# monkey0head/RePlay_cql

Measured on AMD Instinct MI355X. Metric: CQL train-steps/sec, higher is better.
Workload: dtype bf16; 1 GPU; BASELINE.json configs[2]: synthetic 1000000 users x 100000 items, CQL d=128, L=50, B=4096/GPU, bf16 MFMA + fp32 accumulate; users=1000000, items=100000, d=128, window=50, batch_per_gpu=4096, global_batch=4096, parallelism=dp1 (users sharded by rank, RCCL gradient all-reduce), k=10, dp_variant=single

## Files before the change

### replay_cql_amd/csrc/common.h

```cpp
#pragma once
#include <hip/hip_runtime.h>
#include <stdint.h>
#include <stdio.h>
#include <stdarg.h>

#include "../../include/cqlrec.h"

typedef __attribute__((ext_vector_type(8))) __bf16 bf16x8;
typedef __attribute__((ext_vector_type(4))) __bf16 bf16x4;
typedef __attribute__((ext_vector_type(16))) float f32x16;
typedef __attribute__((ext_vector_type(4))) float f32x4;
typedef __attribute__((address_space(3))) bf16x4 lds_bf16x4;

#define CQL_WAVE 64
#define CQL_LOG2E 1.4426950408889634f
#define CQL_LN2 0.6931471805599453f
#define NEG_INF_F (-__builtin_inff())

void cql_set_error(const char* fmt, ...);
#define CQL_REQUIRE(cond, ...)            \
  do {                                    \
    if (!(cond)) {                        \
      cql_set_error(__VA_ARGS__);         \
      return CQLREC_ERR_INVALID;          \
// ... 56 lines not shown
}
__device__ __forceinline__ uint32_t pack_bf16x2(float lo, float hi) {
  return (uint32_t)f32_to_bf16_bits(lo) | ((uint32_t)f32_to_bf16_bits(hi) << 16);
}

__device__ __forceinline__ int mfma_row(int reg, int half) { return (reg & 3) + 8 * (reg >> 2) + 4 * half; }

template <int D>
__device__ __forceinline__ int swz_chunk(int row, int ch) {
  if constexpr (D == 64) return ch ^ ((row >> 1) & 7);
  else return ch ^ (row & 15);
}

__device__ __forceinline__ float fast_exp2(float x) { return __builtin_amdgcn_exp2f(x); }

__device__ __forceinline__ uint32_t f32_order_key(float f) {
  uint32_t u = __float_as_uint(f);
  return (u & 0x80000000u) ? ~u : (u | 0x80000000u);
}
__device__ __forceinline__ float f32_from_order_key(uint32_t k) {
  uint32_t u = (k & 0x80000000u) ? (k & 0x7FFFFFFFu) : ~k;
  return __uint_as_float(u);
}

struct CqlAdamFix {
  int valid;
  const float* slab;
  const float* slab_cs;
  int32_t G, T, nblk, items, D;
  float scale;
  int64_t n_items;
  int64_t rows_off, cs_off;
};
int cql_adam_ema_fix(float* theta, float* grads, float* m, float* v, float* target, uint16_t* theta_b, uint16_t* target_b,
                     int64_t n, float step_size, float sqrt_bc2, float beta1, float beta2, float eps, float tau,
                     int32_t zero_grads, const CqlAdamFix* fix, hipStream_t stream);
#define CQL_ADAM_DEFER_CAP 64
struct CqlAdamSteps {
  float step_size[CQL_ADAM_DEFER_CAP], sqrt_bc2[CQL_ADAM_DEFER_CAP];
};
int cql_adam_ema_rows_deferred(float* theta, float* grads, float* m, float* v, float* target, uint16_t* theta_b,
                               uint16_t* target_b, int64_t n, const CqlAdamSteps& tab, uint64_t step, float beta1, float beta2,
                               float eps, float tau, int32_t zero_grads, const uint8_t* row_map, const uint8_t* read_next,
                               uint8_t* age, int32_t d, int64_t n_rows, hipStream_t stream);
int cql_mark_read_rows(const int64_t* offsets, const int32_t* items, const int32_t* users, const int32_t* tpos,
                       int64_t n_states, int32_t L, int64_t n_items, uint8_t* read_map, hipStream_t s);
int cql_gather_pool_bwd_mark_rows(const void* ws, int64_t n_states, int32_t L, int32_t d, int64_t n_items, uint8_t* row_map,
                                  hipStream_t s);
```

### replay_cql_amd/csrc/gbwd.hip

```cpp
#include <cstring>
#include <rocprim/device/device_radix_sort.hpp>

#include "common.h"

__global__ __launch_bounds__(256) void gbwd_pairs_kernel(const int64_t* __restrict__ offsets,
                                                         const int32_t* __restrict__ items,
                                                         const int32_t* __restrict__ users,
                                                         const int32_t* __restrict__ ends, int end_delta,
                                                         int64_t n_states, int L, uint32_t pad_key,
                                                         uint32_t* __restrict__ keys, uint32_t* __restrict__ vals,
                                                         int32_t* __restrict__ lens) {
  const int lane = threadIdx.x & 63;
  const int64_t state = (int64_t)blockIdx.x * 4 + (threadIdx.x >> 6);
  if (state >= n_states) return;
  const int u = users[state];
  const int64_t o0 = offsets[u];
  const int end = ends ? (ends[state] + end_delta) : (int)(offsets[u + 1] - o0);
  const int len = end < L ? end : L;
  if (lane == 0) lens[state] = len;
  const int32_t* win = items + o0 + end - len;
  for (int j = lane; j < L; j += 64) {
    keys[state * L + j] = (j < len) ? (uint32_t)win[j] : pad_key;
    vals[state * L + j] = (uint32_t)state;
  }
}

__global__ __launch_bounds__(256) void gbwd_scale_kernel(const float4* __restrict__ dh0, const int32_t* __restrict__ lens,
                                                         int64_t n4, int d4, float4* __restrict__ g) {
  const int64_t i = (int64_t)blockIdx.x * blockDim.x + threadIdx.x;
  if (i >= n4) return;
  const int len = lens[i / d4];
  const float fl = (float)len;
  const float4 v = dh0[i];
  g[i] = len > 0 ? make_float4(v.x / fl, v.y / fl, v.z / fl, v.w / fl) : make_float4(0.f, 0.f, 0.f, 0.f);
}

template <int D, bool SRC_BF16>
__device__ __forceinline__ void segsum_add_row(float (&acc)[D / 64], float& accw, const void* __restrict__ src,
                                               const float* __restrict__ w, uint32_t row, int lane) {
  constexpr int PER = D / 64;
  if constexpr (SRC_BF16) {
    const float wt = w[row];
    const uint16_t* h = (const uint16_t*)src + (int64_t)row * D;
#pragma unroll
    for (int k = 0; k < PER; ++k) acc[k] += wt * bf16_bits_to_f32(h[k * 64 + lane]);
    accw += wt;
  } else {
    const float* g = (const float*)src + (int64_t)row * D;
#pragma unroll
    for (int k = 0; k < PER; ++k) acc[k] += g[k * 64 + lane];
  }
}

template <int D, bool SRC_BF16, int CH>
__global__ __launch_bounds__(256) void segsum_pass1_kernel(const void* __restrict__ src, const float* __restrict__ w,
                                                           const uint32_t* __restrict__ keys,
                                                           const uint32_t* __restrict__ vals, int64_t n_pairs,
                                                           uint32_t pad_key, float* __restrict__ dst,
                                                           float* __restrict__ dst_w, float* __restrict__ edge,
                                                           float* __restrict__ edge_w, int accumulate) {
  constexpr int PER = D / 64;
  const int lane = threadIdx.x & 63;
  const int64_t chunk = (int64_t)blockIdx.x * 4 + (threadIdx.x >> 6);
  const int64_t chunk0 = chunk * CH;
  if (chunk0 >= n_pairs) return;
  const int64_t idx = chunk0 + lane;
  const bool mine = lane < CH && idx < n_pairs;
  const uint32_t my_key = mine ? keys[idx] : pad_key;
  const uint32_t my_val = mine ? vals[idx] : 0u;
  if (__builtin_amdgcn_readfirstlane(my_key) == pad_key) return;
  const uint32_t prev_key = (chunk0 > 0) ? keys[chunk0 - 1] : pad_key;
  const uint32_t next_key = (chunk0 + CH < n_pairs) ? keys[chunk0 + CH] : pad_key;
  float acc[PER], accw = 0.f;
#pragma unroll
  for (int k = 0; k < PER; ++k) acc[k] = 0.f;
  uint32_t run_key = __builtin_amdgcn_readfirstlane(my_key);
  bool open_left = (run_key == prev_key);
  auto flush = [&](bool open_right) {
    float* row;
    float* roww = nullptr;
    if (open_left) { row = edge + (chunk * 2 + 0) * D; if (SRC_BF16) roww = edge_w + chunk * 2 + 0; }
    else if (open_right) { row = edge + (chunk * 2 + 1) * D; if (SRC_BF16) roww = edge_w + chunk * 2 + 1; }
    else { row = dst + (int64_t)run_key * D; if (SRC_BF16) roww = dst_w + run_key; }
    const bool add = accumulate && row != edge + (chunk * 2 + 0) * D && row != edge + (chunk * 2 + 1) * D;
#pragma unroll
    for (int k = 0; k < PER; ++k) row[k * 64 + lane] = add ? row[k * 64 + lane] + acc[k] : acc[k];
    if (SRC_BF16 && lane == 0) *roww = add ? *roww + accw : accw;
  };
#pragma unroll 8
  for (int j = 0; j < CH; ++j) {
    const uint32_t kj = __shfl(my_key, j);
    if (kj != run_key) {
      flush(false);
#pragma unroll
      for (int k = 0; k < PER; ++k) acc[k] = 0.f;
      accw = 0.f;
      run_key = kj;
      open_left = false;
      if (kj == pad_key) return;
    }
    segsum_add_row<D, SRC_BF16>(acc, accw, src, w, __shfl(my_val, j), lane);
  }
  flush(run_key == next_key);
}

template <int D, bool SRC_BF16, int CH>
__global__ __launch_bounds__(256) void segsum_pass2_kernel(const uint32_t* __restrict__ keys, int64_t n_pairs,
                                                           uint32_t pad_key, const float* __restrict__ edge,
                                                           const float* __restrict__ edge_w, float* __restrict__ dst,
                                                           float* __restrict__ dst_w, int accumulate) {
  constexpr int PER = D / 64;
  const int lane = threadIdx.x & 63;
  const int64_t c = (int64_t)blockIdx.x * 4 + (threadIdx.x >> 6);
  const int64_t n_chunks = (n_pairs + CH - 1) / CH;
  if (c + 1 >= n_chunks) return;
  auto key_at = [&](int64_t i) { return i < n_pairs ? keys[i] : pad_key; };
  const uint32_t k = key_at(c * CH + CH - 1);
  if (k == pad_key || key_at((c + 1) * CH) != k) return;
  if (key_at(c * CH) == k && c > 0 && key_at(c * CH - 1) == k) return;
  int64_t lo = (c + 1) * CH, hi = n_pairs;
  while (lo < hi) {
    const int64_t mid = (lo + hi) >> 1;
    if (keys[mid] == k) lo = mid + 1; else hi = mid;
  }
  const int64_t j_end = (lo - 1) / CH;
  float acc[PER], accw = 0.f;
#pragma unroll
  for (int q = 0; q < PER; ++q) acc[q] = edge[(c * 2 + 1) * D + q * 64 + lane];
  if (SRC_BF16) accw = edge_w[c * 2 + 1];
#pragma unroll 4
  for (int64_t j = c + 1; j <= j_end; ++j) {
#pragma unroll
    for (int q = 0; q < PER; ++q) acc[q] += edge[(j * 2 + 0) * D + q * 64 + lane];
    if (SRC_BF16) accw += edge_w[j * 2 + 0];
  }
#pragma unroll
  for (int q = 0; q < PER; ++q) {
    float* o = dst + (int64_t)k * D + q * 64 + lane;
    *o = accumulate ? *o + acc[q] : acc[q];
  }
  if (SRC_BF16 && lane == 0) dst_w[k] = accumulate ? dst_w[k] + accw : accw;
}

template <bool SRC_BF16, int CH>
static void segsum_launch(const void* src, const float* w, const uint32_t* keys, const uint32_t* vals, int64_t n_pairs,
                          uint32_t pad_key, int d, float* dst, float* dst_w, float* edge, float* edge_w, hipStream_t s,
                          int accumulate = 0) {
  dim3 grid(cql_ceil_div((n_pairs + CH - 1) / CH, 4)), block(256);
#define SS1(DD) hipLaunchKernelGGL((segsum_pass1_kernel<DD, SRC_BF16, CH>), grid, block, 0, s, src, w, keys, vals, n_pairs, pad_key, dst, dst_w, edge, edge_w, accumulate)
#define SS2(DD) hipLaunchKernelGGL((segsum_pass2_kernel<DD, SRC_BF16, CH>), grid, block, 0, s, keys, n_pairs, pad_key, edge, edge_w, dst, dst_w, accumulate)
  if (d == 64) { SS1(64); SS2(64); } else if (d == 128) { SS1(128); SS2(128); } else { SS1(256); SS2(256); }
#undef SS1
#undef SS2
}

#define GB_CH 64
#define OH_CH 8

static inline int64_t a256(int64_t x) { return (x + 255) / 256 * 256; }
static inline unsigned key_bits(int64_t n_items) {
  unsigned b = 1;
  while ((1ll << b) <= n_items) ++b;
  return b;
}
static int64_t sort_temp_bound(int64_t n) { return a256(2 * n * 4 * 2) + (8ll << 20); }

namespace {
struct GbWs {
  float* g;
  float* edge;
  int32_t* lens;
  uint32_t *keys_in, *vals_in, *keys_out, *vals_out;
  void* temp;
  size_t temp_cap;
  int64_t total;
};
GbWs gb_carve(void* ws, int64_t n_states, int32_t L, int32_t d) {
  const int64_t n = n_states * L;
  char* p = (char*)ws;
  GbWs w;
  w.g = (float*)p;              p += a256(n_states * d * 4);
  w.edge = (float*)p;           p += a256(((n + GB_CH - 1) / GB_CH) * 2 * d * 4);
  w.lens = (int32_t*)p;         p += a256(n_states * 4);
// ... 168 lines not shown
int cql_onehot_prepare(const int32_t* act, int64_t batch, int64_t n_items, int32_t d, void* ws, int64_t ws_bytes,
                       hipStream_t s) {
  CQL_REQUIRE(act && ws, "onehot_prepare: NULL pointer");
  CQL_REQUIRE(batch > 0 && ws_bytes >= cql_onehot_ws_bytes(batch, d), "onehot_prepare: workspace too small");
  const OhWs w = oh_carve(ws, batch, d);
  CqlProfScope prof(CQLREC_PH_GATHER_BWD, s);
  hipLaunchKernelGGL(onehot_pairs_kernel, dim3(cql_ceil_div(batch, 256)), dim3(256), 0, s, act, batch, w.keys_in, w.vals_in);
  size_t need = 0;
  hipError_t e = rocprim::radix_sort_pairs(nullptr, need, w.keys_in, w.keys_out, w.vals_in, w.vals_out, (size_t)batch, 0u,
                                           key_bits(n_items), s);
  if (e != hipSuccess || need > w.temp_cap) {
    cql_set_error("onehot_prepare: radix sort needs %zu bytes of scratch (have %zu), err=%d", need, w.temp_cap, (int)e);
    return CQLREC_ERR_HIP;
  }
  e = rocprim::radix_sort_pairs(w.temp, need, w.keys_in, w.keys_out, w.vals_in, w.vals_out, (size_t)batch, 0u,
                                key_bits(n_items), s);
  if (e != hipSuccess) {
    cql_set_error("onehot_prepare: radix sort failed: %s", hipGetErrorString(e));
    return CQLREC_ERR_HIP;
  }
  CQL_LAUNCH_CHECK("onehot_prepare");
  return CQLREC_OK;
}

int cql_onehot_apply(const float* coef, const uint16_t* H_b, int64_t batch, int64_t n_items, int32_t d, void* ws,
                     float* g_E_out, float* g_b_out, hipStream_t s, int accumulate) {
  CQL_REQUIRE(coef && H_b && ws && g_E_out && g_b_out, "onehot_apply: NULL pointer");
  const OhWs w = oh_carve(ws, batch, d);
  CqlProfScope prof(CQLREC_PH_QHEAD_SMALL, s);
  segsum_launch<true, OH_CH>(H_b, coef, w.keys_out, w.vals_out, batch, (uint32_t)n_items, d, g_E_out, g_b_out, w.edge, w.edge_w, s, accumulate);
  CQL_LAUNCH_CHECK("onehot_apply");
  return CQLREC_OK;
}
```

### replay_cql_amd/csrc/misc.hip

```cpp
#include <stdlib.h>
#include "common.h"
#include "adam_math.h"

static thread_local char g_err[512] = "";
void cql_set_error(const char* fmt, ...) {
  va_list ap;
  va_start(ap, fmt);
  vsnprintf(g_err, sizeof(g_err), fmt, ap);
  va_end(ap);
}
extern "C" const char* cqlrec_last_error(void) { return g_err; }
extern "C" int cqlrec_abi_version(void) { return CQLREC_ABI_VERSION; }

#define CQL_PROF_POOL 8192
static struct {
  bool on = false;
  bool created = false;
  hipEvent_t ev[CQL_PROF_POOL][2];
  int phase[CQL_PROF_POOL];
  int n = 0;
  int open = -1;
  uint32_t mask = 0xFFFFFFFFu;
} g_prof;

// ... 732 lines not shown
      st4<NT>(theta + i, p[0], p[1], p[2], p[3]);
      st4<NT>(m + i, mm[0], mm[1], mm[2], mm[3]);
      st4<NT>(v + i, vv[0], vv[1], vv[2], vv[3]);
      st4<NT>(target + i, tt[0], tt[1], tt[2], tt[3]);
      theta_b[i] = make_uint2(pack_bf16x2(p[0], p[1]), pack_bf16x2(p[2], p[3]));
      target_b[i] = make_uint2(pack_bf16x2(tt[0], tt[1]), pack_bf16x2(tt[2], tt[3]));
    }
    if (zero_grads) st4<NT>(grads + i, 0.f, 0.f, 0.f, 0.f);
  }
}

int cql_adam_ema_rows_deferred(float* theta, float* grads, float* m, float* v, float* target, uint16_t* theta_b,
                               uint16_t* target_b, int64_t n, const CqlAdamSteps& tab, uint64_t step, float beta1, float beta2,
                               float eps, float tau, int32_t zero_grads, const uint8_t* row_map, const uint8_t* read_next,
                               uint8_t* age, int32_t d, int64_t n_rows, hipStream_t stream) {
  CQL_REQUIRE(theta && grads && m && v && target && theta_b && target_b && row_map && age,
              "adam_ema_rows_deferred: NULL pointer");
  CQL_REQUIRE(n > 0 && n % 4 == 0, "adam_ema_rows_deferred: n=%lld must be a positive multiple of 4", (long long)n);
  CQL_REQUIRE(d == 64 || d == 128 || d == 256, "adam_ema_rows_deferred: d=%d unsupported", d);
  CQL_REQUIRE(n_rows >= 0 && n_rows * d <= n, "adam_ema_rows_deferred: %lld rows of %d do not fit n=%lld", (long long)n_rows,
              d, (long long)n);
  const int64_t n4 = n / 4;
  int blocks = (int)((n4 + 255) / 256);
  if (blocks > 8192) blocks = 8192;
  CqlProfScope prof(CQLREC_PH_ADAM, stream);
  hipLaunchKernelGGL(adam_ema_rows_deferred_kernel<true>, dim3(blocks), dim3(256), 0, stream, (float4*)theta, (float4*)grads,
                     (float4*)m, (float4*)v, (float4*)target, (uint2*)theta_b, (uint2*)target_b, n4, tab, (uint32_t)step,
                     beta1, beta2, eps, tau, zero_grads, row_map, read_next, age, __builtin_ctz((unsigned)d) - 2, n_rows);
  CQL_LAUNCH_CHECK("adam_ema (deferred rows)");
  return CQLREC_OK;
}

__device__ __forceinline__ void adam_fix4(const CqlAdamFix& f, float (&g)[4], int64_t i4, int ld, int li) {
  const int64_t e = 4 * i4;
  uint32_t item;
  int col = -1;
  if (e >= f.rows_off && e < f.rows_off + f.n_items * f.D) {
    const uint64_t r = (uint64_t)(e - f.rows_off);
    item = (uint32_t)(r >> ld);
    col = (int)(r & (uint64_t)(f.D - 1));
  } else if (e >= f.cs_off && e < f.cs_off + f.n_items) {
    item = (uint32_t)(e - f.cs_off);
  } else {
    return;
  }
#ifdef ADAMFIX_ABL_NOLOOP
  return;
#endif
  const uint32_t grp = item >> li, row = item & (uint32_t)(f.items - 1);
  const uint32_t W = (uint32_t)f.G * (uint32_t)f.T, nblk = (uint32_t)f.nblk, lo = grp * (uint32_t)f.T, hi = lo + (uint32_t)f.T;
  for (uint32_t p = ((lo + 1) * nblk + W - 1) / W; p < nblk; ++p) {
    const uint32_t u0 = (uint32_t)((uint64_t)p * W / nblk);
    if (u0 >= hi) break;
    if (u0 <= lo) continue;
    if ((uint32_t)(((uint64_t)p + 1) * W / nblk) == u0) continue;
    if (col >= 0) {
      const float4 s4 = *reinterpret_cast<const float4*>(f.slab + ((int64_t)p * f.items + row) * f.D + col);
      g[0] += f.scale * s4.x; g[1] += f.scale * s4.y; g[2] += f.scale * s4.z; g[3] += f.scale * s4.w;
    } else {
      const float* sc = f.slab_cs + (int64_t)p * f.items + row;
#pragma unroll
      for (int k = 0; k < 4; ++k)
        if ((int64_t)item + k < f.n_items) g[k] += f.scale * sc[k];
    }
  }
}

template <bool NT>
__global__ __launch_bounds__(256) void adam_ema_fix_kernel(float4* __restrict__ theta, float4* __restrict__ grads,
                                                           float4* __restrict__ m, float4* __restrict__ v,
                                                           float4* __restrict__ target, uint2* __restrict__ theta_b,
                                                           uint2* __restrict__ target_b, int64_t n4, float step_size,
                                                           float sqrt_bc2, float beta1, float beta2, float eps, float tau,
                                                           int zero_grads, CqlAdamFix fix) {
  const float omb1 = 1.0f - beta1, omb2 = 1.0f - beta2, omt = 1.0f - tau;
  const int ld = __builtin_ctz((unsigned)fix.D), li = __builtin_ctz((unsigned)fix.items);
  for (int64_t i = (int64_t)blockIdx.x * blockDim.x + threadIdx.x; i < n4; i += (int64_t)gridDim.x * blockDim.x) {
    const float4 g4 = ld4<NT>(grads + i);
    float4 p4 = ld4<NT>(theta + i), m4 = ld4<NT>(m + i), v4 = ld4<NT>(v + i), t4 = ld4<NT>(target + i);
    float g[4] = {g4.x, g4.y, g4.z, g4.w};
    adam_fix4(fix, g, i, ld, li);
    float p[4] = {p4.x, p4.y, p4.z, p4.w}, mm[4] = {m4.x, m4.y, m4.z, m4.w}, vv[4] = {v4.x, v4.y, v4.z, v4.w},
          tt[4] = {t4.x, t4.y, t4.z, t4.w};
#pragma unroll
    for (int k = 0; k < 4; ++k) {
      adam_ema_elem(g[k], p[k], mm[k], vv[k], tt[k], step_size, sqrt_bc2, beta1, beta2, eps, tau, omb1, omb2, omt);
    }
    st4<NT>(theta + i, p[0], p[1], p[2], p[3]);
    st4<NT>(m + i, mm[0], mm[1], mm[2], mm[3]);
    st4<NT>(v + i, vv[0], vv[1], vv[2], vv[3]);
    st4<NT>(target + i, tt[0], tt[1], tt[2], tt[3]);
    theta_b[i] = make_uint2(pack_bf16x2(p[0], p[1]), pack_bf16x2(p[2], p[3]));
    target_b[i] = make_uint2(pack_bf16x2(tt[0], tt[1]), pack_bf16x2(tt[2], tt[3]));
    if (zero_grads) st4<NT>(grads + i, 0.f, 0.f, 0.f, 0.f);
  }
}

int cql_adam_ema_fix(float* theta, float* grads, float* m, float* v, float* target, uint16_t* theta_b, uint16_t* target_b,
                     int64_t n, float step_size, float sqrt_bc2, float beta1, float beta2, float eps, float tau,
                     int32_t zero_grads, const CqlAdamFix* fix, hipStream_t stream) {
  const bool pow2 = fix && fix->valid && (fix->D & (fix->D - 1)) == 0 && (fix->items & (fix->items - 1)) == 0 &&
                    fix->rows_off % 4 == 0 && fix->cs_off % 4 == 0 &&
                    (int64_t)fix->G * fix->T * ((int64_t)fix->nblk + 1) < (1ll << 31) && fix->n_items < (1ll << 31);
  CQL_REQUIRE(!fix || !fix->valid || pow2, "adam_ema: deferred fix-up outside the supported range");
  if (!fix || !fix->valid)
    return cqlrec_adam_ema(theta, grads, m, v, target, theta_b, target_b, n, step_size, sqrt_bc2, beta1, beta2, eps, tau,
                           zero_grads, (cqlrec_stream)stream);
  CQL_REQUIRE(theta && grads && m && v && target && theta_b && target_b, "adam_ema: NULL pointer");
  CQL_REQUIRE(n > 0 && n % 4 == 0, "adam_ema: n=%lld must be a positive multiple of 4", (long long)n);
  const int64_t n4 = n / 4;
  int blocks = (int)((n4 + 255) / 256);
  if (blocks > 8192) blocks = 8192;
  CqlProfScope prof(CQLREC_PH_ADAM, stream);
  hipLaunchKernelGGL(adam_ema_fix_kernel<true>, dim3(blocks), dim3(256), 0, stream, (float4*)theta, (float4*)grads,
                     (float4*)m, (float4*)v, (float4*)target, (uint2*)theta_b, (uint2*)target_b, n4, step_size, sqrt_bc2,
                     beta1, beta2, eps, tau, zero_grads, *fix);
  CQL_LAUNCH_CHECK("adam_ema (deferred fix-up)");
  return CQLREC_OK;
}

extern "C" int cqlrec_adam_ema(float* theta, float* grads, float* m, float* v, float* target, uint16_t* theta_b,
                               uint16_t* target_b, int64_t n, float step_size, float sqrt_bc2, float beta1, float beta2,
                               float eps, float tau, int32_t zero_grads, cqlrec_stream stream) {
  CQL_REQUIRE(theta && grads && m && v && target && theta_b && target_b, "adam_ema: NULL pointer");
  CQL_REQUIRE(n > 0 && n % 4 == 0, "adam_ema: n=%lld must be a positive multiple of 4", (long long)n);
  const int64_t n4 = n / 4;
  int blocks = (int)((n4 + 255) / 256);
  if (blocks > 8192) blocks = 8192;
  CqlProfScope prof(CQLREC_PH_ADAM, (hipStream_t)stream);
  hipLaunchKernelGGL(adam_ema_kernel<true>, dim3(blocks), dim3(256), 0, (hipStream_t)stream, (float4*)theta,
                     (float4*)grads, (float4*)m, (float4*)v, (float4*)target, (uint2*)theta_b, (uint2*)target_b, n4,
                     step_size, sqrt_bc2, beta1, beta2, eps, tau, zero_grads);
  CQL_LAUNCH_CHECK("adam_ema");
  return CQLREC_OK;
}

__global__ __launch_bounds__(256) void cast_bf16_kernel(const float4* __restrict__ src, uint2* __restrict__ dst,
                                                        int64_t n4) {
  for (int64_t i = (int64_t)blockIdx.x * blockDim.x + threadIdx.x; i < n4; i += (int64_t)gridDim.x * blockDim.x) {
    const float4 p = src[i];
    dst[i] = make_uint2(pack_bf16x2(p.x, p.y), pack_bf16x2(p.z, p.w));
  }
}
extern "C" int cqlrec_cast_bf16(const float* src, uint16_t* dst_b, int64_t n, cqlrec_stream stream) {
  CQL_REQUIRE(src && dst_b, "cast_bf16: NULL pointer");
  CQL_REQUIRE(n > 0 && n % 4 == 0, "cast_bf16: n=%lld must be a positive multiple of 4", (long long)n);
  const int64_t n4 = n / 4;
  int blocks = (int)((n4 + 255) / 256);
  if (blocks > 8192) blocks = 8192;
// ... 6 lines not shown
```

### replay_cql_amd/csrc/train.hip

```cpp
#include <math.h>
#include <stdlib.h>
#include "common.h"
#include "qhead_internal.h"

static int g_concurrency = -1;

enum { MK_LOSS = 0, MK_DH, MK_DE, MK_CHAIN, MK_ADAM_IN, MK_ADAM_OUT, MK_PROLOGUE, MK_LSE, MK_NEXT_LOSS, MK_ENC_DX, MK_GATHER_BWD, MK_SORT_NEXT, MK_COUNT };
static hipEvent_t g_marks[MK_COUNT];
static int g_marks_on = 0;
static int g_mark_phase = 0;
static void mark(int k, hipStream_t s) {
  if (g_marks_on && g_mark_phase) (void)hipEventRecord(g_marks[k], s);
}
extern "C" int cqlrec_debug_marks_enable(int32_t on) {
  if (on && !g_marks[0])
    for (int i = 0; i < MK_COUNT; ++i)
      if (hipEventCreate(&g_marks[i]) != hipSuccess) return CQLREC_ERR_HIP;
  g_marks_on = on ? 1 : 0;
  return CQLREC_OK;
}
extern "C" int cqlrec_debug_marks_read(float* ms_out) {
  if (!g_marks[0] || !ms_out) return CQLREC_ERR_INVALID;
  for (int i = 0; i < MK_COUNT; ++i) {
    ms_out[i] = -1.f;
    if (hipEventSynchronize(g_marks[i]) != hipSuccess) continue;
    float ms = 0.f;
    if (hipEventElapsedTime(&ms, g_marks[MK_LOSS], g_marks[i]) == hipSuccess) ms_out[i] = ms;
  }
  return CQLREC_OK;
}

namespace {
struct Carve {
  char* base;
  int64_t off;
  explicit Carve(void* p) : base((char*)p), off(0) {}
  template <typename T>
  T* take(int64_t n) {
    T* p = base ? (T*)(base + off) : nullptr;
    off += (n * (int64_t)sizeof(T) + 255) / 256 * 256;
    return p;
  }
};

struct StepWs {
  int32_t *users, *tpos, *act, *a_star;
  float *rew, *done, *q_a, *lse, *nlse2, *nlse_nat, *q_targ, *y, *coef, *maxv, *loss, *term;
  float *h0_s, *dH, *dh0;
  uint16_t *h0b, *zb, *hb, *h0b_t, *zb_t, *hb_t;
  void *ws_q, *ws_q2, *ws_qb, *ws_qb2, *ws_enc, *ws_gb, *ws_oh;
  uint8_t* row_map;
  uint8_t* read_map;
  uint8_t* age;
  int64_t ws_q_bytes, ws_qb_bytes, ws_qf_bytes, ws_enc_bytes, ws_gb_bytes, ws_oh_bytes;
  int64_t total;
};

void carve_small(Carve& c, StepWs& w, int32_t B, int32_t d) {
  w.users = c.take<int32_t>(B);
  w.tpos = c.take<int32_t>(B);
  w.act = c.take<int32_t>(B);
  w.a_star = c.take<int32_t>(B);
  w.rew = c.take<float>(B);
  w.done = c.take<float>(B);
  w.q_a = c.take<float>(B);
  w.lse = c.take<float>(B);
  w.nlse2 = c.take<float>(B);
  w.nlse_nat = c.take<float>(B);
  w.q_targ = c.take<float>(B);
  w.y = c.take<float>(B);
  w.coef = c.take<float>(B);
  w.maxv = c.take<float>(B);
  w.loss = c.take<float>(64);
  w.term = c.take<float>(B);
  w.h0_s = c.take<float>((int64_t)B * d);
  w.dH = c.take<float>((int64_t)B * d);
  w.dh0 = c.take<float>((int64_t)B * d);
  w.h0b = c.take<uint16_t>((int64_t)2 * B * d);
  w.zb = c.take<uint16_t>((int64_t)2 * B * d);
  w.hb = c.take<uint16_t>((int64_t)2 * B * d);
  w.h0b_t = c.take<uint16_t>((int64_t)B * d);
  w.zb_t = c.take<uint16_t>((int64_t)B * d);
  w.hb_t = c.take<uint16_t>((int64_t)B * d);
}

StepWs carve_step(void* ws, int32_t B, int64_t N, int32_t d, int32_t L, uint64_t step = 0) {
  StepWs w, other;
  Carve c(ws);
  if (step & 1) {
    carve_small(c, other, B, d);
    carve_small(c, w, B, d);
  } else {
    carve_small(c, w, B, d);
    carve_small(c, other, B, d);
  }
  w.ws_q_bytes = cqlrec_qhead_ws_bytes(B, N, d);
  w.ws_q = c.take<char>(w.ws_q_bytes);
  w.ws_q2 = c.take<char>(w.ws_q_bytes);
  w.ws_qb_bytes = cqlrec_qhead_bwd_ws_bytes(B, N, d);
  w.ws_qf_bytes = w.ws_qb_bytes + w.ws_q_bytes;
  w.ws_qb = c.take<char>(w.ws_qf_bytes);
  w.ws_qb2 = c.take<char>(w.ws_qb_bytes);
  w.ws_enc_bytes = cqlrec_encoder_bwd_ws_bytes(B, d);
  w.ws_enc = c.take<char>(w.ws_enc_bytes);
  w.ws_gb_bytes = cqlrec_gather_pool_bwd_ws_bytes(B, L, d);
  void* gb0 = c.take<char>(w.ws_gb_bytes);
  void* gb1 = c.take<char>(w.ws_gb_bytes);
  w.ws_gb = (step & 1) ? gb1 : gb0;
  w.ws_oh_bytes = cql_onehot_ws_bytes(B, d);
  void* oh0 = c.take<char>(w.ws_oh_bytes);
  void* oh1 = c.take<char>(w.ws_oh_bytes);
  w.ws_oh = (step & 1) ? oh1 : oh0;
  uint8_t* rm0 = c.take<uint8_t>(N);
  uint8_t* rm1 = c.take<uint8_t>(N);
  w.row_map = (step & 1) ? rm1 : rm0;
  uint8_t* rd0 = c.take<uint8_t>(N);
  uint8_t* rd1 = c.take<uint8_t>(N);
  w.read_map = (step & 1) ? rd1 : rd0;
  w.age = c.take<uint8_t>(N);
  w.total = c.off;
  return w;
}

int check_ctx(const cqlrec_train_ctx* c) {
  CQL_REQUIRE(c != nullptr, "train_step: ctx is NULL");
  CQL_REQUIRE(c->offsets && c->items && c->rewards, "train_step: CSR pointers are NULL");
  CQL_REQUIRE(c->theta && c->grads && c->adam_m && c->adam_v && c->target && c->theta_b && c->target_b,
              "train_step: model state pointers are NULL");
  CQL_REQUIRE(c->ws != nullptr, "train_step: workspace is NULL");
  CQL_REQUIRE(c->batch > 0 && c->window > 0 && c->world > 0 && c->rank >= 0 && c->rank < c->world,
              "train_step: batch=%d window=%d world=%d rank=%d", c->batch, c->window, c->world, c->rank);
  const int32_t d = c->layout.d;
  CQL_REQUIRE(d == 64 || d == 128 || d == 256, "train_step: d=%d unsupported", d);
  CQL_REQUIRE(c->ws_bytes >= cqlrec_train_ws_bytes(c->batch, c->layout.n_items, d, c->window),
              "train_step: workspace too small");
  return CQLREC_OK;
}
}

extern "C" int cqlrec_set_concurrency(int32_t on) {
  g_concurrency = on ? 1 : 0;
  return CQLREC_OK;
}

extern "C" int64_t cqlrec_train_ws_bytes(int32_t batch, int64_t n_items, int32_t d, int32_t window) {
  return carve_step(nullptr, batch, n_items, d, window).total + 256;
}

#define CQL_TRY(expr)            \
  do {                           \
    int rc__ = (expr);           \
    if (rc__ != CQLREC_OK) return rc__; \
// ... 278 lines not shown
  CQL_TRY(cql_qhead_argmax_step(w.hb + Bd, B, p.Eout_b, p.b_out, N, d, w.ws_q2, w.ws_q_bytes, w.maxv, w.a_star, (hipStream_t)sb));
  CQL_TRY(cqlrec_gather_dot(w.hb_t, p.tEout_b, p.tb_out, w.a_star, B, d, w.q_targ, sb));
  if (par && (hipEventRecord(ss.join2, ss.s2) != hipSuccess || hipStreamWaitEvent(s, ss.join2, 0) != hipSuccess)) {
    cql_set_error("train_step_forward: joining the forward branches failed");
    return CQLREC_ERR_HIP;
  }
  const float inv_batch = 1.0f / ((float)B * (float)c->world);
  CQL_TRY(cql_td_coef(w.q_a, w.lse, w.q_targ, w.rew, w.done, B, (float)c->gamma, (float)c->alpha, inv_batch, w.coef, w.y,
                      w.term, s));
  if (loss_sum_deferred) *loss_sum_deferred = true;
  else CQL_TRY(cql_td_loss_sum(w.term, B, inv_batch, loss_out ? loss_out : w.loss, s));
  if (g_mark_phase == 2) mark(MK_NEXT_LOSS, s);
  return CQLREC_OK;
}

int backward_items_long_impl(const cqlrec_train_ctx* c, uint64_t step, cqlrec_stream stream, CqlAdamFix* fix) {
  const cqlrec_layout& L = c->layout;
  const int32_t B = c->batch, d = L.d;
  StepWs w = carve_step(c->ws, B, L.n_items, d, c->window, step);
  const StepPtrs p = step_ptrs(c);
  return cql_qhead_bwd_items_long(w.hb, w.nlse2, w.coef, w.act, B, p.Eout_b, p.b_out, L.n_items, d, alpha_scale(c), w.ws_qb2,
                                  w.ws_qb_bytes, c->grads + L.off_E_out, c->grads + L.off_b_out, (hipStream_t)stream, fix,
                                  w.nlse_nat);
}
int backward_items_onehot_impl(const cqlrec_train_ctx* c, uint64_t step, cqlrec_stream stream) {
  const cqlrec_layout& L = c->layout;
  const int32_t B = c->batch, d = L.d;
  StepWs w = carve_step(c->ws, B, L.n_items, d, c->window, step);
  SideStream& ss = side_stream();
  if (ss.ok) CQL_HIP_TRY(hipStreamWaitEvent((hipStream_t)stream, ss.sorted[step & 1], 0), "train_step_backward_items");
  return cql_onehot_apply(w.coef, w.hb, B, L.n_items, d, w.ws_oh, c->grads + L.off_E_out, c->grads + L.off_b_out,
                          (hipStream_t)stream, 1);
}
int backward_items_impl(const cqlrec_train_ctx* c, uint64_t step, cqlrec_stream stream, CqlAdamFix* defer = nullptr) {
  const cqlrec_layout& L = c->layout;
  CqlAdamFix fix = {};
  CQL_TRY(backward_items_long_impl(c, step, stream, &fix));
  CQL_TRY(backward_items_onehot_impl(c, step, stream));
  if (defer) *defer = fix;
  else CQL_TRY(cql_qde_fixup_deferred(fix, c->grads + L.off_E_out, c->grads + L.off_b_out, (hipStream_t)stream));
  return CQLREC_OK;
}

int backward_states_impl(const cqlrec_train_ctx* c, uint64_t step, cqlrec_stream stream) {
  const cqlrec_layout& L = c->layout;
  const int32_t B = c->batch, d = L.d;
  const int64_t N = L.n_items;
  StepWs w = carve_step(c->ws, B, N, d, c->window, step);
  const StepPtrs p = step_ptrs(c);
  CQL_TRY(cql_qhead_dh_finish(w.ws_qb, B, N, d, w.lse, w.coef, w.act, p.Eout_b, alpha_scale(c), w.dH,
                              (hipStream_t)stream, 2));
  SideStream& ss = side_stream();
  if (ss.ok) CQL_HIP_TRY(hipEventRecord(ss.dh, (hipStream_t)stream), "train_step_backward_rest");
  return CQLREC_OK;
}

int backward_chain_impl(const cqlrec_train_ctx* c, uint64_t step, cqlrec_stream stream) {
  const cqlrec_layout& L = c->layout;
  const int32_t B = c->batch, d = L.d, W = c->window;
  const int64_t N = L.n_items;
  StepWs w = carve_step(c->ws, B, N, d, W, step);
  const StepPtrs p = step_ptrs(c);
  SideStream& ss = side_stream();
  hipStream_t s = (hipStream_t)stream;
  const bool split = ss.ok && ss.s2 && ss.s2 != s;
  CQL_TRY(cql_encoder_bwd_parts(w.dH, w.zb, w.h0b, p.W1_b, p.W2_b, B, d, w.ws_enc, w.ws_enc_bytes, c->grads + L.off_W1,
// ... 50 lines not shown
extern "C" int cqlrec_train_step_backward_items(const cqlrec_train_ctx* c, uint64_t step, cqlrec_stream stream) {
  CQL_TRY(check_ctx(c));
  if (g_early_long[step & 1]) {
    g_early_long[step & 1] = false;
    const cqlrec_layout& L = c->layout;
    CQL_TRY(backward_items_onehot_impl(c, step, stream));
    return cql_qde_fixup_deferred(g_early_fix[step & 1], c->grads + L.off_E_out, c->grads + L.off_b_out, (hipStream_t)stream);
  }
  return backward_items_impl(c, step, stream);
}

extern "C" int cqlrec_train_step_backward_rest(const cqlrec_train_ctx* c, uint64_t step, cqlrec_stream stream) {
  CQL_TRY(check_ctx(c));
  return backward_rest_impl(c, step, stream);
}

extern "C" int cqlrec_train_step_fwd_bwd(const cqlrec_train_ctx* c, uint64_t step, float* loss_out,
                                         cqlrec_stream stream) {
  CQL_TRY(cqlrec_train_step_forward(c, step, loss_out, stream));
  SideStream& ss = side_stream();
  hipStream_t s = (hipStream_t)stream;
  if (need_side_streams(ss) && hipEventRecord(ss.loss, s) == hipSuccess && hipStreamWaitEvent(ss.s, ss.loss, 0) == hipSuccess) {
    CQL_TRY(backward_items_impl(c, step, (cqlrec_stream)ss.s));
    CQL_HIP_TRY(hipEventRecord(ss.items, ss.s), "train_step_fwd_bwd");
    CQL_TRY(backward_rest_impl(c, step, stream));
    CQL_HIP_TRY(hipStreamWaitEvent(s, ss.items, 0), "train_step_fwd_bwd");
    return CQLREC_OK;
  }
  CQL_TRY(backward_rest_impl(c, step, stream));
  return backward_items_impl(c, step, stream);
}

int update_range_impl(const cqlrec_train_ctx* c, uint64_t step, int64_t lo, int64_t hi, cqlrec_stream stream,
                      const CqlAdamFix* fix, int zero_grads = 1);
namespace {
void adam_step_scalars(const cqlrec_train_ctx* c, uint64_t step, float* step_size, float* sqrt_bc2) {
  const double t = (double)(step + 1);
  const double bc1 = 1.0 - pow((double)c->beta1, t);
  const double bc2 = 1.0 - pow((double)c->beta2, t);
  *step_size = (float)((double)c->lr / bc1);
  *sqrt_bc2 = (float)sqrt(bc2);
}
}
extern "C" int cqlrec_train_steps(const cqlrec_train_ctx* c, uint64_t step0, int32_t n_steps, float* loss_out,
                                  cqlrec_stream stream) {
  CQL_TRY(check_ctx(c));
  CQL_REQUIRE(n_steps >= 0, "train_steps: n_steps=%d", n_steps);
  CQL_REQUIRE(c->world == 1, "train_steps: world=%d; data-parallel callers use the phase entry points", c->world);
  const cqlrec_layout& L = c->layout;
  hipStream_t s = (hipStream_t)stream;
  hipEvent_t pending = nullptr;
  hipEvent_t sampled = nullptr;
  need_side_streams(side_stream(), true);
  const bool use_map = n_steps > 1 && L.off_E_in == 0;
  CqlAdamSteps adam_tab = {};
  if (use_map) {
    const StepWs w0 = carve_step(c->ws, c->batch, L.n_items, L.d, c->window, step0);
    CQL_HIP_TRY(hipMemsetAsync(w0.age, 0, (size_t)L.n_items, s), "train_steps");
  }
  bool grads_dirty = false;
  for (int32_t i = 0; i < n_steps; ++i) {
    const uint64_t step = step0 + (uint64_t)i;
    const bool lean = use_map && i + 1 < n_steps;
    static const int early_de = !(getenv("CQL_EARLY_DE") && getenv("CQL_EARLY_DE")[0] == '0');
    SideStream& ss0 = side_stream();
    const bool early = early_de && ss0.ok && ss0.s;
    CqlAdamFix fix = {};
    bool sum_deferred = false;
    const bool can_defer = ss0.ok && ss0.s3 && i + 1 < n_steps;
    CQL_TRY(forward_impl(c, step, loss_out ? loss_out + i : nullptr, stream, pending, sampled, early ? ss0.s : nullptr, &fix,
                         can_defer ? &sum_deferred : nullptr, use_map));
    pending = sampled = nullptr;
    if (g_marks_on && n_steps >= 4) {
      if (i == n_steps / 2) g_mark_phase = 1;
      else if (i == n_steps / 2 + 1) g_mark_phase = 0;
    }
    SideStream& ss = side_stream();
    if (g_mark_phase == 1) mark(MK_LOSS, s);
    if (ss.ok && hipEventRecord(ss.loss, s) == hipSuccess) {
      if (i + 1 < n_steps && hipStreamWaitEvent(ss.s3, ss.loss, 0) == hipSuccess) {
        if (sum_deferred) {
          CQL_TRY(loss_sum_impl(c, step, loss_out ? loss_out + i : nullptr, ss.s3));
          sum_deferred = false;
        }
        CQL_TRY(sample_ahead(c, step + 1, (cqlrec_stream)ss.s3, ss.presample, ss.read_map));
        CQL_HIP_TRY(hipEventRecord(ss.sorted[(step + 1) & 1], ss.s3), "train_steps");
        if (g_mark_phase == 1) mark(MK_SORT_NEXT, ss.s3);
        sampled = ss.presample;
      }
      if (sum_deferred) CQL_TRY(loss_sum_impl(c, step, loss_out ? loss_out + i : nullptr, s));
      CQL_HIP_TRY(hipStreamWaitEvent(ss.s, ss.loss, 0), "train_steps");
      if (early)
        CQL_TRY(backward_items_onehot_impl(c, step, (cqlrec_stream)ss.s));
      else
        CQL_TRY(backward_items_impl(c, step, (cqlrec_stream)ss.s, &fix));
      if (g_mark_phase == 1) mark(MK_DE, ss.s);
      CQL_TRY(backward_states_impl(c, step, stream));
      if (g_mark_phase == 1) mark(MK_DH, s);
      CQL_TRY(backward_chain_impl(c, step, stream));
      if (g_mark_phase == 1) mark(MK_CHAIN, s);
      CQL_TRY(cqlrec_train_step_update_range(c, step, L.off_W1, L.total, stream));
      if (use_map) {
        const StepWs w = carve_step(c->ws, c->batch, L.n_items, L.d, c->window, step);
        const int slot = (int)(step % CQL_ADAM_DEFER_CAP);
        adam_step_scalars(c, step, &adam_tab.step_size[slot], &adam_tab.sqrt_bc2[slot]);
        const uint8_t* read_next = nullptr;
        if (lean && sampled) {
          CQL_HIP_TRY(hipStreamWaitEvent(s, ss.read_map, 0), "train_steps");
          read_next = carve_step(c->ws, c->batch, L.n_items, L.d, c->window, step + 1).read_map;
        }
        CQL_TRY(cql_adam_ema_rows_deferred(c->theta, c->grads, c->adam_m, c->adam_v, c->target, c->theta_b, c->target_b,
                                           L.off_E_out, adam_tab, step, (float)c->beta1, (float)c->beta2, (float)c->eps,
                                           (float)c->tau, lean ? 0 : 1, w.row_map, read_next, w.age, L.d, L.n_items, s));
      } else {
        CQL_TRY(cqlrec_train_step_update_range(c, step, 0, L.off_E_out, stream));
      }
      if (g_mark_phase == 1) mark(MK_ADAM_IN, s);
      CQL_HIP_TRY(hipStreamWaitEvent(ss.s, ss.dh, 0), "train_steps");
      fix.rows_off = 0;
      fix.cs_off = L.off_b_out - L.off_E_out;
      CQL_TRY(update_range_impl(c, step, L.off_E_out, L.off_W1, (cqlrec_stream)ss.s, &fix, lean ? 0 : 1));
      grads_dirty = lean;
      CQL_HIP_TRY(hipEventRecord(ss.eout, ss.s), "train_steps");
      if (g_mark_phase == 1) { mark(MK_ADAM_OUT, ss.s); g_mark_phase = 2; }
      pending = ss.eout;
    } else {
      CQL_REQUIRE(!grads_dirty, "train_steps: lost the side streams in the middle of a call");
      if (sum_deferred) CQL_TRY(loss_sum_impl(c, step, loss_out ? loss_out + i : nullptr, s));
      CQL_TRY(backward_rest_impl(c, step, stream));
      CQL_TRY(backward_items_impl(c, step, stream));
      CQL_TRY(cqlrec_train_step_update_range(c, step, 0, L.total, stream));
    }
  }
  g_mark_phase = 0;
  if (pending) CQL_HIP_TRY(hipStreamWaitEvent(s, pending, 0), "train_steps");
  return CQLREC_OK;
}

extern "C" int cqlrec_train_step_update_range(const cqlrec_train_ctx* c, uint64_t step, int64_t lo, int64_t hi,
                                              cqlrec_stream stream) {
  return update_range_impl(c, step, lo, hi, stream, nullptr);
}

int update_range_impl(const cqlrec_train_ctx* c, uint64_t step, int64_t lo, int64_t hi, cqlrec_stream stream,
                      const CqlAdamFix* fix, int zero_grads) {
  CQL_TRY(check_ctx(c));
  CQL_REQUIRE(lo >= 0 && hi <= c->layout.total && lo < hi && lo % 4 == 0 && hi % 4 == 0,
              "train_step_update_range: bad range [%lld, %lld)", (long long)lo, (long long)hi);
  float step_size, sqrt_bc2;
  adam_step_scalars(c, step, &step_size, &sqrt_bc2);
  return cql_adam_ema_fix(c->theta + lo, c->grads + lo, c->adam_m + lo, c->adam_v + lo, c->target + lo, c->theta_b + lo,
                          c->target_b + lo, hi - lo, step_size, sqrt_bc2, (float)c->beta1, (float)c->beta2, (float)c->eps,
                          (float)c->tau, zero_grads, fix, (hipStream_t)stream);
}

extern "C" int cqlrec_train_step_update(const cqlrec_train_ctx* c, uint64_t step, cqlrec_stream stream) {
  CQL_TRY(check_ctx(c));
  return cqlrec_train_step_update_range(c, step, 0, c->layout.total, stream);
}

extern "C" int cqlrec_train_views_get(const cqlrec_train_ctx* c, uint64_t step, cqlrec_train_views* out) {
  CQL_TRY(check_ctx(c));
  CQL_REQUIRE(out != nullptr, "train_views_get: out is NULL");
  const int32_t B = c->batch, d = c->layout.d;
  StepWs w = carve_step(c->ws, B, c->layout.n_items, d, c->window, step);
  out->users = w.users; out->tpos = w.tpos; out->act = w.act; out->a_star = w.a_star;
  out->rew = w.rew; out->done = w.done; out->q_a = w.q_a; out->lse = w.lse; out->q_targ = w.q_targ;
  out->y = w.y; out->coef = w.coef; out->dH = w.dH; out->dh0 = w.dh0; out->h0_s = w.h0_s;
  out->hb_s = w.hb; out->hb_sn = w.hb + (int64_t)B * d; out->hb_tn = w.hb_t;
  return CQLREC_OK;
}
```

Before: 1555 train-steps/s (B=4096 transitions per step and GPU).

## Fold one-hot output-embedding gradient sums into the Adam update via compact tagged map

Instead of scattering per-item one-hot gradient sums into the dense output-embedding gradient buffer, the segmented-sum kernels now write compact per-run rows plus a tagged item->slot map. The fused Adam/EMA kernel reads the map and adds those sums while it streams the embedding rows, which removes a separate read-modify-write of the scattered gradient rows. In exchange, the Adam kernel does an extra map lookup per 4-element group over the whole item table, and the map must be memset once per call.

```diff
diff --git a/replay_cql_amd/csrc/common.h b/replay_cql_amd/csrc/common.h
--- a/replay_cql_amd/csrc/common.h
+++ b/replay_cql_amd/csrc/common.h
@@ -112,9 +112,21 @@
   int64_t n_items;
   int64_t rows_off, cs_off;
 };
+struct CqlAdamOnehot {
+  int valid;
+  const float* rows;
+  const float* bias;
+  const uint2* map;
+  uint32_t tag;
+  int32_t D;
+  int64_t n_items;
+  int64_t rows_off, cs_off;
+};
+int cql_onehot_sums(const float* coef, const uint16_t* H_b, int64_t batch, int64_t n_items, int32_t d, void* ws, float* rows,
+                    float* bias, uint2* map, uint32_t tag, hipStream_t s);
 int cql_adam_ema_fix(float* theta, float* grads, float* m, float* v, float* target, uint16_t* theta_b, uint16_t* target_b,
                      int64_t n, float step_size, float sqrt_bc2, float beta1, float beta2, float eps, float tau,
-                     int32_t zero_grads, const CqlAdamFix* fix, hipStream_t stream);
+                     int32_t zero_grads, const CqlAdamFix* fix, hipStream_t stream, const CqlAdamOnehot* onehot = nullptr);
 #define CQL_ADAM_DEFER_CAP 64
 struct CqlAdamSteps {
   float step_size[CQL_ADAM_DEFER_CAP], sqrt_bc2[CQL_ADAM_DEFER_CAP];
diff --git a/replay_cql_amd/csrc/gbwd.hip b/replay_cql_amd/csrc/gbwd.hip
--- a/replay_cql_amd/csrc/gbwd.hip
+++ b/replay_cql_amd/csrc/gbwd.hip
@@ -52,13 +52,14 @@
   }
 }
 
-template <int D, bool SRC_BF16, int CH>
+template <int D, bool SRC_BF16, int CH, bool COMPACT = false>
 __global__ __launch_bounds__(256) void segsum_pass1_kernel(const void* __restrict__ src, const float* __restrict__ w,
                                                            const uint32_t* __restrict__ keys,
                                                            const uint32_t* __restrict__ vals, int64_t n_pairs,
                                                            uint32_t pad_key, float* __restrict__ dst,
                                                            float* __restrict__ dst_w, float* __restrict__ edge,
-                                                           float* __restrict__ edge_w, int accumulate) {
+                                                           float* __restrict__ edge_w, int accumulate,
+                                                           uint2* __restrict__ map = nullptr, uint32_t tag = 0) {
   constexpr int PER = D / 64;
   const int lane = threadIdx.x & 63;
   const int64_t chunk = (int64_t)blockIdx.x * 4 + (threadIdx.x >> 6);
@@ -76,11 +77,17 @@
   for (int k = 0; k < PER; ++k) acc[k] = 0.f;
   uint32_t run_key = __builtin_amdgcn_readfirstlane(my_key);
   bool open_left = (run_key == prev_key);
+  int64_t run_start = chunk0;
   auto flush = [&](bool open_right) {
     float* row;
     float* roww = nullptr;
     if (open_left) { row = edge + (chunk * 2 + 0) * D; if (SRC_BF16) roww = edge_w + chunk * 2 + 0; }
     else if (open_right) { row = edge + (chunk * 2 + 1) * D; if (SRC_BF16) roww = edge_w + chunk * 2 + 1; }
+    else if constexpr (COMPACT) {
+      row = dst + run_start * D;
+      if (SRC_BF16) roww = dst_w + run_start;
+      if (lane == 0) map[run_key] = make_uint2(tag, (uint32_t)run_start);
+    }
     else { row = dst + (int64_t)run_key * D; if (SRC_BF16) roww = dst_w + run_key; }
     const bool add = accumulate && row != edge + (chunk * 2 + 0) * D && row != edge + (chunk * 2 + 1) * D;
 #pragma unroll
@@ -97,6 +104,7 @@
       accw = 0.f;
       run_key = kj;
       open_left = false;
+      run_start = chunk0 + j;
       if (kj == pad_key) return;
     }
     segsum_add_row<D, SRC_BF16>(acc, accw, src, w, __shfl(my_val, j), lane);
@@ -104,11 +112,12 @@
   flush(run_key == next_key);
 }
 
-template <int D, bool SRC_BF16, int CH>
+template <int D, bool SRC_BF16, int CH, bool COMPACT = false>
 __global__ __launch_bounds__(256) void segsum_pass2_kernel(const uint32_t* __restrict__ keys, int64_t n_pairs,
                                                            uint32_t pad_key, const float* __restrict__ edge,
                                                            const float* __restrict__ edge_w, float* __restrict__ dst,
-                                                           float* __restrict__ dst_w, int accumulate) {
+                                                           float* __restrict__ dst_w, int accumulate,
+                                                           uint2* __restrict__ map = nullptr, uint32_t tag = 0) {
   constexpr int PER = D / 64;
   const int lane = threadIdx.x & 63;
   const int64_t c = (int64_t)blockIdx.x * 4 + (threadIdx.x >> 6);
@@ -134,6 +143,16 @@
     for (int q = 0; q < PER; ++q) acc[q] += edge[(j * 2 + 0) * D + q * 64 + lane];
     if (SRC_BF16) accw += edge_w[j * 2 + 0];
   }
+  if constexpr (COMPACT) {
+    const int64_t slot = c * CH + CH - 1;
+#pragma unroll
+    for (int q = 0; q < PER; ++q) dst[slot * D + q * 64 + lane] = acc[q];
+    if (lane == 0) {
+      if (SRC_BF16) dst_w[slot] = accw;
+      map[k] = make_uint2(tag, (uint32_t)slot);
+    }
+    return;
+  }
 #pragma unroll
   for (int q = 0; q < PER; ++q) {
     float* o = dst + (int64_t)k * D + q * 64 + lane;
@@ -142,13 +161,13 @@
   if (SRC_BF16 && lane == 0) dst_w[k] = accumulate ? dst_w[k] + accw : accw;
 }
 
-template <bool SRC_BF16, int CH>
+template <bool SRC_BF16, int CH, bool COMPACT = false>
 static void segsum_launch(const void* src, const float* w, const uint32_t* keys, const uint32_t* vals, int64_t n_pairs,
                           uint32_t pad_key, int d, float* dst, float* dst_w, float* edge, float* edge_w, hipStream_t s,
-                          int accumulate = 0) {
+                          int accumulate = 0, uint2* map = nullptr, uint32_t tag = 0) {
   dim3 grid(cql_ceil_div((n_pairs + CH - 1) / CH, 4)), block(256);
-#define SS1(DD) hipLaunchKernelGGL((segsum_pass1_kernel<DD, SRC_BF16, CH>), grid, block, 0, s, src, w, keys, vals, n_pairs, pad_key, dst, dst_w, edge, edge_w, accumulate)
-#define SS2(DD) hipLaunchKernelGGL((segsum_pass2_kernel<DD, SRC_BF16, CH>), grid, block, 0, s, keys, n_pairs, pad_key, edge, edge_w, dst, dst_w, accumulate)
+#define SS1(DD) hipLaunchKernelGGL((segsum_pass1_kernel<DD, SRC_BF16, CH, COMPACT>), grid, block, 0, s, src, w, keys, vals, n_pairs, pad_key, dst, dst_w, edge, edge_w, accumulate, map, tag)
+#define SS2(DD) hipLaunchKernelGGL((segsum_pass2_kernel<DD, SRC_BF16, CH, COMPACT>), grid, block, 0, s, keys, n_pairs, pad_key, edge, edge_w, dst, dst_w, accumulate, map, tag)
   if (d == 64) { SS1(64); SS2(64); } else if (d == 128) { SS1(128); SS2(128); } else { SS1(256); SS2(256); }
 #undef SS1
 #undef SS2
@@ -383,3 +402,14 @@
   CQL_LAUNCH_CHECK("onehot_apply");
   return CQLREC_OK;
 }
+
+int cql_onehot_sums(const float* coef, const uint16_t* H_b, int64_t batch, int64_t n_items, int32_t d, void* ws, float* rows,
+                    float* bias, uint2* map, uint32_t tag, hipStream_t s) {
+  CQL_REQUIRE(coef && H_b && ws && rows && bias && map, "onehot_sums: NULL pointer");
+  CQL_REQUIRE(tag != 0, "onehot_sums: tag 0 is the cleared map's");
+  const OhWs w = oh_carve(ws, batch, d);
+  CqlProfScope prof(CQLREC_PH_QHEAD_SMALL, s);
+  segsum_launch<true, OH_CH, true>(H_b, coef, w.keys_out, w.vals_out, batch, (uint32_t)n_items, d, rows, bias, w.edge, w.edge_w, s, 0, map, tag);
+  CQL_LAUNCH_CHECK("onehot_sums");
+  return CQLREC_OK;
+}
diff --git a/replay_cql_amd/csrc/misc.hip b/replay_cql_amd/csrc/misc.hip
--- a/replay_cql_amd/csrc/misc.hip
+++ b/replay_cql_amd/csrc/misc.hip
@@ -788,6 +788,7 @@
 }
 
 __device__ __forceinline__ void adam_fix4(const CqlAdamFix& f, float (&g)[4], int64_t i4, int ld, int li) {
+  if (!f.valid) return;
   const int64_t e = 4 * i4;
   uint32_t item;
   int col = -1;
@@ -822,19 +823,42 @@
   }
 }
 
+__device__ __forceinline__ void adam_onehot4(const CqlAdamOnehot& o, float (&g)[4], int64_t i4, int ld) {
+  if (!o.valid) return;
+  const int64_t e = 4 * i4;
+  if (e >= o.rows_off && e < o.rows_off + o.n_items * o.D) {
+    const uint64_t r = (uint64_t)(e - o.rows_off);
+    const uint2 ent = o.map[r >> ld];
+    if (ent.x == o.tag) {
+      const float4 s4 = *reinterpret_cast<const float4*>(o.rows + (((int64_t)ent.y) << ld) + (int64_t)(r & (uint64_t)(o.D - 1)));
+      g[0] += s4.x; g[1] += s4.y; g[2] += s4.z; g[3] += s4.w;
+    }
+  } else if (e >= o.cs_off && e < o.cs_off + o.n_items) {
+    const int64_t item = e - o.cs_off;
+#pragma unroll
+    for (int k = 0; k < 4; ++k)
+      if (item + k < o.n_items) {
+        const uint2 ent = o.map[item + k];
+        if (ent.x == o.tag) g[k] += o.bias[ent.y];
+      }
+  }
+}
+
 template <bool NT>
 __global__ __launch_bounds__(256) void adam_ema_fix_kernel(float4* __restrict__ theta, float4* __restrict__ grads,
                                                            float4* __restrict__ m, float4* __restrict__ v,
                                                            float4* __restrict__ target, uint2* __restrict__ theta_b,
                                                            uint2* __restrict__ target_b, int64_t n4, float step_size,
                                                            float sqrt_bc2, float beta1, float beta2, float eps, float tau,
-                                                           int zero_grads, CqlAdamFix fix) {
+                                                           int zero_grads, CqlAdamFix fix, CqlAdamOnehot oh) {
   const float omb1 = 1.0f - beta1, omb2 = 1.0f - beta2, omt = 1.0f - tau;
-  const int ld = __builtin_ctz((unsigned)fix.D), li = __builtin_ctz((unsigned)fix.items);
+  const int ld = fix.valid ? __builtin_ctz((unsigned)fix.D) : 0, li = fix.valid ? __builtin_ctz((unsigned)fix.items) : 0;
+  const int ld_oh = oh.valid ? __builtin_ctz((unsigned)oh.D) : 0;
   for (int64_t i = (int64_t)blockIdx.x * blockDim.x + threadIdx.x; i < n4; i += (int64_t)gridDim.x * blockDim.x) {
     const float4 g4 = ld4<NT>(grads + i);
     float4 p4 = ld4<NT>(theta + i), m4 = ld4<NT>(m + i), v4 = ld4<NT>(v + i), t4 = ld4<NT>(target + i);
     float g[4] = {g4.x, g4.y, g4.z, g4.w};
+    adam_onehot4(oh, g, i, ld_oh);
     adam_fix4(fix, g, i, ld, li);
     float p[4] = {p4.x, p4.y, p4.z, p4.w}, mm[4] = {m4.x, m4.y, m4.z, m4.w}, vv[4] = {v4.x, v4.y, v4.z, v4.w},
           tt[4] = {t4.x, t4.y, t4.z, t4.w};
@@ -854,12 +878,20 @@
 
 int cql_adam_ema_fix(float* theta, float* grads, float* m, float* v, float* target, uint16_t* theta_b, uint16_t* target_b,
                      int64_t n, float step_size, float sqrt_bc2, float beta1, float beta2, float eps, float tau,
-                     int32_t zero_grads, const CqlAdamFix* fix, hipStream_t stream) {
+                     int32_t zero_grads, const CqlAdamFix* fix, hipStream_t stream, const CqlAdamOnehot* onehot) {
+  const bool has_oh = onehot && onehot->valid;
+  if (has_oh) {
+    CQL_REQUIRE(onehot->rows && onehot->bias && onehot->map && onehot->tag != 0, "adam_ema: one-hot sums without buffers");
+    CQL_REQUIRE(onehot->D >= 4 && (onehot->D & (onehot->D - 1)) == 0 && onehot->rows_off % 4 == 0 && onehot->cs_off % 4 == 0 &&
+                    onehot->n_items > 0 && onehot->rows_off >= 0 && onehot->rows_off + onehot->n_items * onehot->D <= n &&
+                    onehot->cs_off >= 0 && onehot->cs_off + onehot->n_items <= n,
+                "adam_ema: one-hot sums outside the updated range");
+  }
   const bool pow2 = fix && fix->valid && (fix->D & (fix->D - 1)) == 0 && (fix->items & (fix->items - 1)) == 0 &&
                     fix->rows_off % 4 == 0 && fix->cs_off % 4 == 0 &&
                     (int64_t)fix->G * fix->T * ((int64_t)fix->nblk + 1) < (1ll << 31) && fix->n_items < (1ll << 31);
   CQL_REQUIRE(!fix || !fix->valid || pow2, "adam_ema: deferred fix-up outside the supported range");
-  if (!fix || !fix->valid)
+  if ((!fix || !fix->valid) && !has_oh)
     return cqlrec_adam_ema(theta, grads, m, v, target, theta_b, target_b, n, step_size, sqrt_bc2, beta1, beta2, eps, tau,
                            zero_grads, (cqlrec_stream)stream);
   CQL_REQUIRE(theta && grads && m && v && target && theta_b && target_b, "adam_ema: NULL pointer");
@@ -870,7 +902,8 @@
   CqlProfScope prof(CQLREC_PH_ADAM, stream);
   hipLaunchKernelGGL(adam_ema_fix_kernel<true>, dim3(blocks), dim3(256), 0, stream, (float4*)theta, (float4*)grads,
                      (float4*)m, (float4*)v, (float4*)target, (uint2*)theta_b, (uint2*)target_b, n4, step_size, sqrt_bc2,
-                     beta1, beta2, eps, tau, zero_grads, *fix);
+                     beta1, beta2, eps, tau, zero_grads, (fix && fix->valid) ? *fix : CqlAdamFix{},
+                     has_oh ? *onehot : CqlAdamOnehot{});
   CQL_LAUNCH_CHECK("adam_ema (deferred fix-up)");
   return CQLREC_OK;
 }
diff --git a/replay_cql_amd/csrc/train.hip b/replay_cql_amd/csrc/train.hip
--- a/replay_cql_amd/csrc/train.hip
+++ b/replay_cql_amd/csrc/train.hip
@@ -52,6 +52,8 @@
   uint8_t* row_map;
   uint8_t* read_map;
   uint8_t* age;
+  uint2* oh_map;
+  float *oh_rows, *oh_bias;
   int64_t ws_q_bytes, ws_qb_bytes, ws_qf_bytes, ws_enc_bytes, ws_gb_bytes, ws_oh_bytes;
   int64_t total;
 };
@@ -118,6 +120,9 @@
   uint8_t* rd1 = c.take<uint8_t>(N);
   w.read_map = (step & 1) ? rd1 : rd0;
   w.age = c.take<uint8_t>(N);
+  w.oh_map = c.take<uint2>(N);
+  w.oh_rows = c.take<float>((int64_t)B * d);
+  w.oh_bias = c.take<float>(B);
   w.total = c.off;
   return w;
 }
@@ -462,6 +467,25 @@
   return cql_onehot_apply(w.coef, w.hb, B, L.n_items, d, w.ws_oh, c->grads + L.off_E_out, c->grads + L.off_b_out,
                           (hipStream_t)stream, 1);
 }
+uint32_t onehot_tag(uint64_t step) { return ((uint32_t)step & 0x7fffffffu) + 1u; }
+int backward_items_onehot_sums_impl(const cqlrec_train_ctx* c, uint64_t step, hipStream_t stream, CqlAdamOnehot* out) {
+  const cqlrec_layout& L = c->layout;
+  const int32_t B = c->batch, d = L.d;
+  StepWs w = carve_step(c->ws, B, L.n_items, d, c->window, step);
+  SideStream& ss = side_stream();
+  if (ss.ok) CQL_HIP_TRY(hipStreamWaitEvent(stream, ss.sorted[step & 1], 0), "train_steps");
+  CQL_TRY(cql_onehot_sums(w.coef, w.hb, B, L.n_items, d, w.ws_oh, w.oh_rows, w.oh_bias, w.oh_map, onehot_tag(step), stream));
+  out->valid = 1;
+  out->rows = w.oh_rows;
+  out->bias = w.oh_bias;
+  out->map = w.oh_map;
+  out->tag = onehot_tag(step);
+  out->D = d;
+  out->n_items = L.n_items;
+  out->rows_off = 0;
+  out->cs_off = L.off_b_out - L.off_E_out;
+  return CQLREC_OK;
+}
 int backward_items_impl(const cqlrec_train_ctx* c, uint64_t step, cqlrec_stream stream, CqlAdamFix* defer = nullptr) {
   const cqlrec_layout& L = c->layout;
   CqlAdamFix fix = {};
@@ -578,7 +602,7 @@
 }
 
 int update_range_impl(const cqlrec_train_ctx* c, uint64_t step, int64_t lo, int64_t hi, cqlrec_stream stream,
-                      const CqlAdamFix* fix, int zero_grads = 1);
+                      const CqlAdamFix* fix, int zero_grads = 1, const CqlAdamOnehot* onehot = nullptr);
 namespace {
 void adam_step_scalars(const cqlrec_train_ctx* c, uint64_t step, float* step_size, float* sqrt_bc2) {
   const double t = (double)(step + 1);
@@ -600,18 +624,22 @@
   need_side_streams(side_stream(), true);
   const bool use_map = n_steps > 1 && L.off_E_in == 0;
   CqlAdamSteps adam_tab = {};
-  if (use_map) {
+  static const int early_de = !(getenv("CQL_EARLY_DE") && getenv("CQL_EARLY_DE")[0] == '0');
+  const bool oh_in_adam = n_steps > 1 && early_de && side_stream().ok && side_stream().s;
+  if (use_map || oh_in_adam) {
     const StepWs w0 = carve_step(c->ws, c->batch, L.n_items, L.d, c->window, step0);
-    CQL_HIP_TRY(hipMemsetAsync(w0.age, 0, (size_t)L.n_items, s), "train_steps");
+    char* lo = use_map ? (char*)w0.age : (char*)w0.oh_map;
+    char* hi = oh_in_adam ? (char*)(w0.oh_map + L.n_items) : (char*)w0.age + L.n_items;
+    CQL_HIP_TRY(hipMemsetAsync(lo, 0, (size_t)(hi - lo), s), "train_steps");
   }
   bool grads_dirty = false;
   for (int32_t i = 0; i < n_steps; ++i) {
     const uint64_t step = step0 + (uint64_t)i;
     const bool lean = use_map && i + 1 < n_steps;
-    static const int early_de = !(getenv("CQL_EARLY_DE") && getenv("CQL_EARLY_DE")[0] == '0');
     SideStream& ss0 = side_stream();
     const bool early = early_de && ss0.ok && ss0.s;
     CqlAdamFix fix = {};
+    CqlAdamOnehot oh = {};
     bool sum_deferred = false;
     const bool can_defer = ss0.ok && ss0.s3 && i + 1 < n_steps;
     CQL_TRY(forward_impl(c, step, loss_out ? loss_out + i : nullptr, stream, pending, sampled, early ? ss0.s : nullptr, &fix,
@@ -624,6 +652,7 @@
     SideStream& ss = side_stream();
     if (g_mark_phase == 1) mark(MK_LOSS, s);
     if (ss.ok && hipEventRecord(ss.loss, s) == hipSuccess) {
+      const bool oh_now = oh_in_adam && early;
       if (i + 1 < n_steps && hipStreamWaitEvent(ss.s3, ss.loss, 0) == hipSuccess) {
         if (sum_deferred) {
           CQL_TRY(loss_sum_impl(c, step, loss_out ? loss_out + i : nullptr, ss.s3));
@@ -636,7 +665,9 @@
       }
       if (sum_deferred) CQL_TRY(loss_sum_impl(c, step, loss_out ? loss_out + i : nullptr, s));
       CQL_HIP_TRY(hipStreamWaitEvent(ss.s, ss.loss, 0), "train_steps");
-      if (early)
+      if (oh_now)
+        CQL_TRY(backward_items_onehot_sums_impl(c, step, ss.s, &oh));
+      else if (early)
         CQL_TRY(backward_items_onehot_impl(c, step, (cqlrec_stream)ss.s));
       else
         CQL_TRY(backward_items_impl(c, step, (cqlrec_stream)ss.s, &fix));
@@ -665,7 +696,7 @@
       CQL_HIP_TRY(hipStreamWaitEvent(ss.s, ss.dh, 0), "train_steps");
       fix.rows_off = 0;
       fix.cs_off = L.off_b_out - L.off_E_out;
-      CQL_TRY(update_range_impl(c, step, L.off_E_out, L.off_W1, (cqlrec_stream)ss.s, &fix, lean ? 0 : 1));
+      CQL_TRY(update_range_impl(c, step, L.off_E_out, L.off_W1, (cqlrec_stream)ss.s, &fix, lean ? 0 : 1, &oh));
       grads_dirty = lean;
       CQL_HIP_TRY(hipEventRecord(ss.eout, ss.s), "train_steps");
       if (g_mark_phase == 1) { mark(MK_ADAM_OUT, ss.s); g_mark_phase = 2; }
@@ -689,7 +720,7 @@
 }
 
 int update_range_impl(const cqlrec_train_ctx* c, uint64_t step, int64_t lo, int64_t hi, cqlrec_stream stream,
-                      const CqlAdamFix* fix, int zero_grads) {
+                      const CqlAdamFix* fix, int zero_grads, const CqlAdamOnehot* onehot) {
   CQL_TRY(check_ctx(c));
   CQL_REQUIRE(lo >= 0 && hi <= c->layout.total && lo < hi && lo % 4 == 0 && hi % 4 == 0,
               "train_step_update_range: bad range [%lld, %lld)", (long long)lo, (long long)hi);
@@ -697,7 +728,7 @@
   adam_step_scalars(c, step, &step_size, &sqrt_bc2);
   return cql_adam_ema_fix(c->theta + lo, c->grads + lo, c->adam_m + lo, c->adam_v + lo, c->target + lo, c->theta_b + lo,
                           c->target_b + lo, hi - lo, step_size, sqrt_bc2, (float)c->beta1, (float)c->beta2, (float)c->eps,
-                          (float)c->tau, zero_grads, fix, (hipStream_t)stream);
+                          (float)c->tau, zero_grads, fix, (hipStream_t)stream, onehot);
 }
 
 extern "C" int cqlrec_train_step_update(const cqlrec_train_ctx* c, uint64_t step, cqlrec_stream stream) {
```

After: 1549 train-steps/s (B=4096 transitions per step and GPU). No clear change (-0.4%).
